# szaguldo-kamaz/FRI-ReinforcementLearning-C

Hardware: AMD Instinct MI355X
Metric: rule-distance evals/sec (rules x envs) (higher is better)
Workload: dtype f64; 1 GPU; cfg4_acrobot_64k_x_8k_per_gpu; nant=5, universe_len=41, rules_per_env=65536, envs_per_gpu=8192, exact_hits=4, dist_backend=none, world_size=1

## Files before the change

### fri-reinforcementlearning-c_amd/__init__.py

```python
import ctypes as C
import os

PKG_DIR = os.path.dirname(os.path.abspath(__file__))
ROOT = os.path.dirname(PKG_DIR)
HIP_LIB_PATH = os.environ.get("FRIRL_HIP_LIB_OVERRIDE") or os.path.join(PKG_DIR, "lib", "libfrirl_hip.so")

NO_HIT = 0xFFFFFFFF
MAX_NANT = 16
MAX_ACTIONS = 32


class FrirlHipError(RuntimeError):
    pass


class Tables(C.Structure):
    _fields_ = [("nant", C.c_int32), ("U", C.c_int32), ("u", C.c_void_p), ("ve", C.c_void_p)]


class RuleBases(C.Structure):
    _fields_ = [("E", C.c_int32), ("maxR", C.c_int32), ("rb", C.c_void_p), ("nrules", C.c_void_p), ("uidx", C.c_void_p)]


MAX_GRID = 64
# ... 29 lines not shown
class ReduceResult(C.Structure):
    _fields_ = [("rules_before", C.c_int32), ("rules_after", C.c_int32), ("rounds", C.c_int32), ("rollouts", C.c_int32),
                ("steps_incremental", C.c_int32), ("reserved", C.c_int32), ("reward", C.c_double)]


class AgentIO(C.Structure):
    _fields_ = [("obs", C.c_void_p), ("q_obs", C.c_void_p), ("reward", C.c_void_p), ("success", C.c_void_p), ("reset", C.c_void_p),
                ("action_out", C.c_void_p), ("action_idx", C.c_void_p)]


class ConvergenceDesc(C.Structure):
    _fields_ = [("prev_nrules", C.c_void_p), ("prev_steps", C.c_void_p), ("prev_reward", C.c_void_p), ("prev_rconc", C.c_void_p),
                ("converged", C.c_void_p), ("episodes", C.c_void_p), ("epended", C.c_void_p)]


_lib = None
_DP = C.POINTER(C.c_double)
LEARN_CHUNK_FN = C.CFUNCTYPE(None, C.c_void_p, C.c_int32, C.c_void_p, C.c_int32)

SIGNATURES = {
    "frirl_hip_version": (C.c_char_p, []),
    "frirl_hip_last_error": (C.c_char_p, []),
    "frirl_hip_device_count": (C.c_int, []),
    "frirl_hip_device_info": (C.c_int, [C.c_int, C.c_char_p, C.c_int, C.POINTER(C.c_int32), C.POINTER(C.c_int64)]),
    "frirl_hip_set_option": (C.c_int, [C.c_char_p, C.c_int]),
    "frirl_hip_get_option": (C.c_int, [C.c_char_p, C.POINTER(C.c_int)]),
    "five_hip_rule_distance_uses_uidx": (C.c_int, [C.c_int32, C.c_int32]),
    "frirl_hip_step_uses_uidx": (C.c_int, [C.c_int32, C.c_int32, C.c_int32, C.c_int32]),
    "five_hip_rule_distance": (C.c_int, [C.POINTER(Tables), C.POINTER(RuleBases), C.c_void_p, C.c_void_p, C.c_void_p, C.c_void_p]),
    "five_hip_rule_distance_packed_words": (C.c_int, [C.c_int32, C.c_int32]),
    "frirl_hip_pack_indices": (C.c_int, [C.POINTER(Tables), C.POINTER(RuleBases), C.c_void_p, C.c_void_p]),
    "five_hip_rule_distance_packed": (C.c_int, [C.POINTER(Tables), C.POINTER(RuleBases), C.c_void_p, C.c_void_p, C.c_void_p, C.c_void_p,
                                                C.c_void_p]),
    "five_hip_sqrt_unscaled_check": (C.c_int, [C.c_void_p, C.c_void_p, C.c_void_p, C.c_int64, C.c_void_p]),
    "five_hip_rule_distance_sq_guard": (C.c_int, [C.POINTER(Tables), C.c_int32, C.c_void_p, C.c_void_p, C.c_void_p]),
    "five_hip_vag_concl": (C.c_int, [C.POINTER(Tables), C.POINTER(RuleBases), C.c_int, C.c_void_p, C.c_void_p, C.c_void_p, C.c_void_p]),
    "five_hip_vag_concl_weight": (C.c_int, [C.POINTER(Tables), C.POINTER(RuleBases), C.c_int, C.c_void_p, C.c_void_p, C.c_void_p, C.c_void_p]),
    "frirl_hip_get_best_action": (C.c_int, [C.POINTER(Tables), C.POINTER(RuleBases), C.c_int, C.c_void_p, C.c_void_p, C.c_int,
                                            C.c_void_p, C.c_void_p, C.c_void_p]),
    "five_hip_vag_concl_shared": (C.c_int, [C.POINTER(Tables), C.POINTER(RuleBases), C.c_int, C.c_int32, C.c_void_p, C.c_void_p, C.c_void_p, C.c_void_p]),
    "frirl_hip_get_best_action_shared": (C.c_int, [C.POINTER(Tables), C.POINTER(RuleBases), C.c_int, C.c_int32, C.c_void_p, C.c_void_p, C.c_int,
                                                   C.c_void_p, C.c_void_p, C.c_void_p]),
    "frirl_hip_rollout_shared": (C.c_int, [C.POINTER(Tables), C.POINTER(RuleBases), C.POINTER(AgentDesc), C.c_int32, C.POINTER(RolloutDesc), C.c_void_p]),
    "frirl_hip_reduce_shared": (C.c_int, [C.POINTER(Tables), C.POINTER(RuleBases), C.POINTER(AgentDesc), C.c_void_p, C.c_int, C.c_double, C.c_int,
                                          C.POINTER(C.c_int32), C.POINTER(ReduceResult), C.c_void_p]),
    "frirl_hip_lanes_preferred": (C.c_int, [C.c_int32, C.c_int32, C.c_int32]),
    "frirl_hip_lanes_workspace_bytes": (C.c_size_t, [C.c_int32, C.c_int32, C.c_int32, C.c_int32]),
    "frirl_hip_episode_run_lanes": (C.c_int, [C.POINTER(Tables), C.POINTER(RuleBases), C.POINTER(AgentDesc), C.POINTER(EnvsDesc), C.c_int32,
                                              C.c_void_p, C.c_size_t, C.c_void_p]),
    "frirl_hip_rollout_resident_rules": (C.c_int, [C.c_int32, C.c_int32, C.c_int32, C.c_int32]),
    "frirl_hip_learn_supported": (C.c_int, [C.c_int32, C.c_int32, C.c_int32, C.c_int32, C.c_int32]),
    "frirl_hip_learn_plan": (C.c_int, [C.c_int32, C.c_int32, C.POINTER(C.c_int32), C.POINTER(C.c_int32)]),
    "frirl_hip_learn_workspace_bytes": (C.c_size_t, [C.c_int32, C.c_int32, C.c_int32, C.c_int32]),
    "frirl_hip_learn_run": (C.c_int, [C.POINTER(Tables), C.POINTER(RuleBases), C.POINTER(AgentDesc), C.POINTER(EnvsDesc), C.POINTER(ConvergenceDesc),
                                      C.c_void_p, C.c_int32, C.c_int32, C.c_int32, C.c_void_p, C.c_void_p, C.c_void_p, C.c_size_t, C.c_void_p]),
    "frirl_hip_learn_train_workspace_bytes": (C.c_size_t, [C.c_int32, C.c_int32, C.c_int32, C.c_int32]),
    "frirl_hip_learn_train": (C.c_int, [C.POINTER(Tables), C.POINTER(RuleBases), C.POINTER(AgentDesc), C.POINTER(EnvsDesc), C.POINTER(ConvergenceDesc),
                                        C.c_int32, C.c_int32, C.c_void_p, C.c_void_p, C.c_void_p, C.c_void_p, C.c_size_t, C.POINTER(C.c_int32),
                                        LEARN_CHUNK_FN, C.c_void_p, C.c_void_p]),
    "five_hip_add_rule": (C.c_int, [C.POINTER(Tables), C.POINTER(RuleBases), C.c_void_p, C.c_void_p, C.c_void_p, C.c_void_p, C.c_void_p,
                                    C.c_void_p]),
    "frirl_hip_update_sarsa": (C.c_int, [C.POINTER(Tables), C.POINTER(RuleBases), C.POINTER(AgentDesc), C.POINTER(EnvsDesc), C.c_void_p,
                                         C.c_void_p, C.c_void_p, C.c_void_p, C.c_void_p]),
    "frirl_hip_env_step": (C.c_int, [C.POINTER(AgentDesc), C.c_int32, C.c_int32, C.c_void_p, C.c_void_p, C.c_void_p, C.c_void_p, C.c_void_p,
                                     C.c_void_p, C.c_void_p]),
    "frirl_hip_episode_begin": (C.c_int, [C.POINTER(Tables), C.POINTER(RuleBases), C.POINTER(AgentDesc), C.POINTER(EnvsDesc), C.c_void_p]),
# ... 89 lines not shown
def _ptr(t):
    return None if t is None else C.c_void_p(t.data_ptr())


def _stream(stream=None):
    import torch
    s = stream if stream is not None else torch.cuda.current_stream()
    return C.c_void_p(s.cuda_stream)


class Problem:

    def __init__(self, u, ve, rb, nrules, uidx=None):
        import torch
        assert u.is_cuda and ve.is_cuda and rb.is_cuda and nrules.is_cuda
        assert u.dtype == torch.float64 and ve.dtype == torch.float64 and rb.dtype == torch.float64 and nrules.dtype == torch.int32
        self.nant, self.U = u.shape
        self.E, cols, self.maxR = rb.shape
        assert cols == self.nant + 1 and ve.shape == u.shape and nrules.shape == (self.E,)
        self.u, self.ve, self.rb, self.nrules = u.contiguous(), ve.contiguous(), rb.contiguous(), nrules.contiguous()
        self.uidx = None
        if uidx is not None:
            assert uidx.is_cuda and uidx.dtype == torch.int16 and uidx.shape == (self.E, self.nant, self.maxR) and self.U <= 32767
            self.uidx = uidx.contiguous()
        self.tables = Tables(self.nant, self.U, self.u.data_ptr(), self.ve.data_ptr())
        self._bases = RuleBases(self.E, self.maxR, self.rb.data_ptr(), self.nrules.data_ptr(),
                                self.uidx.data_ptr() if self.uidx is not None else None)
        self.pidx = None
        self._pidx_key = None
        W = lib().five_hip_rule_distance_packed_words(self.nant, self.U) if self.uidx is not None else 0
        if W > 0:
            self.pidx = torch.empty((self.E, W, self.maxR), dtype=torch.int32, device=self.uidx.device)
            self._pack(None)

    @property
    def bases(self):
        self._pidx_key = None
        return self._bases

    def _pack(self, stream):
        check(lib().frirl_hip_pack_indices(C.byref(self.tables), C.byref(self._bases), _ptr(self.pidx), _stream(stream)),
              "frirl_hip_pack_indices")
        self._pidx_key = (self.uidx.data_ptr(), self.uidx._version)

    def _pidx_current(self, stream):
        if self._pidx_key != (self.uidx.data_ptr(), self.uidx._version):
            self._pack(stream)
        return self.pidx

    def rule_distance(self, x, ruledists=None, hit=None, materialise=True, stream=None):
        import torch
        assert x.is_cuda and x.dtype == torch.float64 and x.shape == (self.E, self.nant) and x.is_contiguous()
        if materialise and ruledists is None:
            ruledists = torch.empty((self.E, self.maxR), dtype=torch.float64, device=x.device)
        if hit is None:
            hit = torch.empty((self.E,), dtype=torch.int32, device=x.device)
        if self.pidx is not None:
            rc = lib().five_hip_rule_distance_packed(C.byref(self.tables), C.byref(self._bases), _ptr(self._pidx_current(stream)), _ptr(x),
                                                     _ptr(ruledists) if materialise else None, _ptr(hit), _stream(stream))
            check(rc, "five_hip_rule_distance_packed")
        else:
            rc = lib().five_hip_rule_distance(C.byref(self.tables), C.byref(self._bases), _ptr(x),
                                              _ptr(ruledists) if materialise else None, _ptr(hit), _stream(stream))
            check(rc, "five_hip_rule_distance")
        return (ruledists if materialise else None), hit

    def vag_concl(self, x, p=0, stream=None):
        import torch
        assert x.is_cuda and x.dtype == torch.float64 and x.shape == (self.E, self.nant) and x.is_contiguous()
        conc = torch.empty((self.E,), dtype=torch.float64, device=x.device)
        hit = torch.empty((self.E,), dtype=torch.int32, device=x.device)
        check(lib().five_hip_vag_concl(C.byref(self.tables), C.byref(self._bases), p, _ptr(x), _ptr(conc), _ptr(hit), _stream(stream)),
              "five_hip_vag_concl")
        return conc, hit

    def vag_concl_weight(self, x, p=0, weights=None, stream=None):
        import torch
        assert x.is_cuda and x.dtype == torch.float64 and x.shape == (self.E, self.nant) and x.is_contiguous()
        if weights is None:
            weights = torch.full((self.E, self.maxR), float("nan"), dtype=torch.float64, device=x.device)
        hit = torch.empty((self.E,), dtype=torch.int32, device=x.device)
        check(lib().five_hip_vag_concl_weight(C.byref(self.tables), C.byref(self._bases), p, _ptr(x), _ptr(weights), _ptr(hit),
                                              _stream(stream)), "five_hip_vag_concl_weight")
        return weights, hit

    def get_best_action(self, states, action_ve, p=0, stream=None):
        import torch
        assert states.is_cuda and states.dtype == torch.float64 and states.shape == (self.E, self.nant - 1) and states.is_contiguous()
        A = action_ve.numel()
        actconc = torch.empty((self.E, A), dtype=torch.float64, device=states.device)
        best = torch.empty((self.E,), dtype=torch.int32, device=states.device)
        check(lib().frirl_hip_get_best_action(C.byref(self.tables), C.byref(self._bases), p, _ptr(states), _ptr(action_ve), A,
                                              _ptr(actconc), _ptr(best), _stream(stream)), "frirl_hip_get_best_action")
# ... 484 lines not shown
```

### fri-reinforcementlearning-c_amd/csrc/device_common.h

```cpp
#pragma once

#include <hip/hip_runtime.h>
#include <stdint.h>

#include "../../include/frirl_hip.h"

#define FRIRL_WAVE 64
#define FRIRL_BLOCK 256
#define FRIRL_WAVES_PER_BLOCK (FRIRL_BLOCK / FRIRL_WAVE)

namespace frirl {

__device__ __forceinline__ unsigned snap_index(const double *__restrict__ uni, int len, double point, double div)
{
    const int low = (int)((point - uni[0]) / div);
    if (low < 0) return 0u;
    if (low >= len) return (unsigned)(len - 1);
    if (low + 1 >= len) return (unsigned)low;
    const double d1 = uni[low] - point;
    const double d2 = uni[low + 1] - point;
    return (fabs(d1) <= fabs(d2)) ? (unsigned)low : (unsigned)(low + 1);
}

__device__ __forceinline__ double universe_div(const double *__restrict__ uni, int U)
// ... 88 lines not shown
    for (int w = 1; w < FRIRL_WAVES_PER_BLOCK; w++) s = s + scratch[w];
    __syncthreads();
    return s;
}

}

namespace frirl_host {
void set_error(const char *fmt, ...);
int check_device();
int check_launch(const char *what);
int check_tables(const frirl_hip_tables *t);
int check_rulebases(const frirl_hip_tables *t, const frirl_hip_rulebases *b);
inline hipStream_t as_stream(void *s) { return reinterpret_cast<hipStream_t>(s); }

struct DeviceGuard {
    int prev = -1;
    DeviceGuard() { if (hipGetDevice(&prev) != hipSuccess) { prev = -1; (void)hipGetLastError(); } }
    ~DeviceGuard() { if (prev >= 0) (void)hipSetDevice(prev); }
    DeviceGuard(const DeviceGuard &) = delete;
    DeviceGuard &operator=(const DeviceGuard &) = delete;
};

struct Options {
    int no_uidx;
    int rd_unroll;
    int rd_chunk;
    int rd_nt;
    int rd_persist;
    int rd_order;
    int rd_packed;
    int rd_sqdiff;
    int rd_qpass;
    int step_wave;
    int step_track;
    int lanes_slices;
    int lanes_wpe;
    int rollout_group;
    int rollout_slices;
    int rollout_resident;
    int rollout_cap;
    int rollout_pair;
    int rollout_wps;
    int learn_slices;
    int learn_alone;
    int learn_persistent;
    int multi_loopback;
    int mirror_sync;
    int no_many;
};
const Options &opts();
}
```

### fri-reinforcementlearning-c_amd/csrc/five_rule_distance.hip

```cpp
#include <stdlib.h>

#include <type_traits>

#include "device_common.h"

namespace frirl {

__device__ __forceinline__ void item_to_env_chunk(unsigned item, int cpe, int E, bool env_fastest, int &e, int &c)
{
    if (env_fastest) { c = (int)(item / (unsigned)E); e = (int)(item - (unsigned)c * (unsigned)E); }
    else { e = (int)(item / (unsigned)cpe); c = (int)(item - (unsigned)e * (unsigned)cpe); }
}

template <int NANT, bool WRITE, int UNROLL, int NT>
__global__ __launch_bounds__(FRIRL_BLOCK) void rule_distance_kernel(
    const double *__restrict__ u, const double *__restrict__ ve, int U, const double *__restrict__ rb,
    const int32_t *__restrict__ nrules, int maxR, const double *__restrict__ x, double *__restrict__ dists,
    uint32_t *__restrict__ hit, int rules_per_block, int cpe, int E, int env_fastest)
{
    int e, c;
    item_to_env_chunk(blockIdx.x, cpe, E, env_fastest != 0, e, c);
    const int R = nrules[e];
    const int r0 = c * rules_per_block;
    if (r0 >= R) return;
// ... 109 lines not shown

    for (int r = r0 + 2 * (int)threadIdx.x; r < r_end; r += STEP * UNROLL) {
        uint32_t w[UNROLL][NANT];
#pragma unroll
        for (int j = 0; j < UNROLL; j++) {
            const int rr = r + j * STEP;
            if (rr < r_end) {
#pragma unroll
                for (int k = 0; k < NANT; k++) w[j][k] = __builtin_nontemporal_load(reinterpret_cast<const uint32_t *>(base + (size_t)k * maxR + rr));
            }
        }
#pragma unroll
        for (int j = 0; j < UNROLL; j++) {
            const int rr = r + j * STEP;
            if (rr < r_end) {
                const double2 d = idx_pair_distance<NANT>(w[j], q, tab_s, U);
                if (WRITE) { __builtin_nontemporal_store(d.x, out + rr); __builtin_nontemporal_store(d.y, out + rr + 1); }
                if (d.y == 0.0 && rr + 1 < R) best = min(best, (unsigned)(rr + 1));
                if (d.x == 0.0) best = min(best, (unsigned)rr);
            }
        }
    }
    best = wave_min_u32(best);
    if ((threadIdx.x & (FRIRL_WAVE - 1)) == 0) red_s[threadIdx.x / FRIRL_WAVE] = best;
    __syncthreads();
    if (threadIdx.x == 0) {
        unsigned m = red_s[0];
        for (int w = 1; w < BLOCK / FRIRL_WAVE; w++) m = red_s[w] < m ? red_s[w] : m;
        if (m != FRIRL_HIP_NO_HIT) atomicMin(&hit[e], m);
    }
}

typedef uint32_t u32x2_t __attribute__((ext_vector_type(2)));

template <int BITS>
__device__ __forceinline__ double pk_table_entry(const double *__restrict__ tab_k, uint32_t w, int sh)
{
    constexpr uint32_t FM = ((1u << BITS) - 1u) << 3;
    const uint32_t off = (sh >= 3 ? (w >> (sh - 3)) : (w << (3 - sh))) & FM;
    return *reinterpret_cast<const double *>(reinterpret_cast<const char *>(tab_k) + off);
}

template <int NANT, int BITS>
__device__ __forceinline__ double2 pk_pair_distance(const u32x2_t (&w)[Packed<BITS>::words(NANT)], const double (&q)[NANT],
                                                    const double *__restrict__ tab_s)
{
    constexpr int FPW = Packed<BITS>::FPW, TS = 1 << BITS;
    double d0 = q[0] - pk_table_entry<BITS>(tab_s, w[0].x, 0), d1 = q[0] - pk_table_entry<BITS>(tab_s, w[0].y, 0);
    double a0 = d0 * d0, a1 = d1 * d1;
#pragma unroll
    for (int k = 1; k < NANT; k++) {
        const int sh = BITS * (k % FPW);
        d0 = q[k] - pk_table_entry<BITS>(tab_s + k * TS, w[k / FPW].x, sh);
        d1 = q[k] - pk_table_entry<BITS>(tab_s + k * TS, w[k / FPW].y, sh);
        const double s0 = d0 * d0, s1 = d1 * d1;
        a0 = a0 + s0;
        a1 = a1 + s1;
    }
    double2 d;
    d.x = __dsqrt_rn(a0);
    d.y = __dsqrt_rn(a1);
    return d;
}

__device__ __forceinline__ double sqrt_unscaled(double x)
{
// ... 11 lines not shown
}

__device__ __forceinline__ bool sq_in_unscaled_range(double s)
{
    return s == 0.0 || (s >= 0x1p-767 && s <= 0x1p1000);
}

template <int NANT, int BITS, bool FAST>
__device__ __forceinline__ void pk_pair_sq(const u32x2_t (&w)[Packed<BITS>::words(NANT)], const double *__restrict__ sq_s, double2 &d,
                                           bool &z0, bool &z1)
{
    constexpr int FPW = Packed<BITS>::FPW, TS = 1 << BITS;
    double a0 = pk_table_entry<BITS>(sq_s, w[0].x, 0), a1 = pk_table_entry<BITS>(sq_s, w[0].y, 0);
#pragma unroll
    for (int k = 1; k < NANT; k++) {
        const int sh = BITS * (k % FPW);
        a0 = a0 + pk_table_entry<BITS>(sq_s + k * TS, w[k / FPW].x, sh);
        a1 = a1 + pk_table_entry<BITS>(sq_s + k * TS, w[k / FPW].y, sh);
    }
    if (FAST) {
        d.x = sqrt_unscaled(a0);
        d.y = sqrt_unscaled(a1);
        z0 = a0 == 0.0;
        z1 = a1 == 0.0;
    } else {
        d.x = __dsqrt_rn(a0);
        d.y = __dsqrt_rn(a1);
        z0 = d.x == 0.0;
        z1 = d.y == 0.0;
    }
}

template <int NANT, int BITS, int BLOCK>
__device__ __forceinline__ bool fill_sq_table(const double *q_s, double *sq_s, const double (&tv)[(NANT * (1 << BITS) + BLOCK - 1) / BLOCK])
{
    constexpr int TS = 1 << BITS, N = NANT * TS;
    bool ok = true;
#pragma unroll
    for (int m = 0; m < (N + BLOCK - 1) / BLOCK; m++) {
        const int i = (int)threadIdx.x + m * BLOCK;
        if (N % BLOCK == 0 || i < N) {
            const double d = q_s[i >> BITS] - tv[m];
            const double s = d * d;
            sq_s[i] = s;
            ok = ok && sq_in_unscaled_range(s);
        }
    }
    return ok;
}

template <int NANT, int BITS, int BLOCK>
__device__ __forceinline__ void load_sq_sources(const double *__restrict__ ve, int U, double (&tv)[(NANT * (1 << BITS) + BLOCK - 1) / BLOCK])
{
    constexpr int TS = 1 << BITS, N = NANT * TS;
#pragma unroll
    for (int m = 0; m < (N + BLOCK - 1) / BLOCK; m++) {
        const int i = (int)threadIdx.x + m * BLOCK;
        const int k = i >> BITS, j = i & (TS - 1);
        tv[m] = (i < N && j < U) ? ve[k * U + j] : 0.0;
    }
}

template <int NANT, bool WRITE, int UNROLL, int BITS, bool SQ>
__global__ __launch_bounds__(FRIRL_BLOCK) void rule_distance_pk_kernel(
    const double *__restrict__ u, const double *__restrict__ ve, int U, const uint32_t *__restrict__ pidx,
    const int32_t *__restrict__ nrules, int maxR, const double *__restrict__ x, const double *__restrict__ qv, double *__restrict__ dists,
    uint32_t *__restrict__ hit, int rules_per_block, int cpe, int E, int env_fastest)
{
    constexpr int W = Packed<BITS>::words(NANT), TS = 1 << BITS;
    __shared__ double tab_s[NANT * TS];
    __shared__ double q_s[NANT];
    __shared__ unsigned red_s[FRIRL_WAVES_PER_BLOCK];
    int e, c;
    item_to_env_chunk(blockIdx.x, cpe, E, env_fastest != 0, e, c);
    const int R = nrules[e];
    const int r0 = c * rules_per_block;
    if (r0 >= R) return;
    int r_end = r0 + rules_per_block;
    if (r_end > R) r_end = R;

    const uint32_t *__restrict__ base = pidx + (size_t)e * W * maxR;
    constexpr int STEP = FRIRL_BLOCK * 2;
    u32x2_t w[UNROLL][W];
    auto load = [&](int r) {
#pragma unroll
        for (int j = 0; j < UNROLL; j++) {
            const int rr = r + j * STEP;
            if (rr < r_end) {
#pragma unroll
                for (int k = 0; k < W; k++) w[j][k] = __builtin_nontemporal_load(reinterpret_cast<const u32x2_t *>(base + (size_t)k * maxR + rr));
            }
        }
    };
    int r = r0 + 2 * (int)threadIdx.x;
    load(r);
    double *__restrict__ out = WRITE ? dists + (size_t)e * maxR : nullptr;
    unsigned best = FRIRL_HIP_NO_HIT;

    if constexpr (SQ) {
        double *sq_s = tab_s;
        double tv[(NANT * TS + FRIRL_BLOCK - 1) / FRIRL_BLOCK];
        load_sq_sources<NANT, BITS, FRIRL_BLOCK>(ve, U, tv);
        if (threadIdx.x < NANT)
            q_s[threadIdx.x] = qv ? qv[(size_t)e * NANT + threadIdx.x] : observe_ve(u, ve, U, threadIdx.x, x[(size_t)e * NANT + threadIdx.x]);
        __syncthreads();
        const bool fast = !__syncthreads_or(!fill_sq_table<NANT, BITS, FRIRL_BLOCK>(q_s, sq_s, tv));
        auto sweep = [&](auto fast_tag) {
            constexpr bool FAST = decltype(fast_tag)::value;
            for (; r < r_end; r += STEP * UNROLL) {
                if (r != r0 + 2 * (int)threadIdx.x) load(r);
#pragma unroll
                for (int j = 0; j < UNROLL; j++) {
                    const int rr = r + j * STEP;
                    if (rr < r_end) {
                        double2 d;
                        bool z0, z1;
                        pk_pair_sq<NANT, BITS, FAST>(w[j], sq_s, d, z0, z1);
                        if (WRITE) { __builtin_nontemporal_store(d.x, out + rr); __builtin_nontemporal_store(d.y, out + rr + 1); }
                        if (z1 && rr + 1 < R) best = min(best, (unsigned)(rr + 1));
                        if (z0) best = min(best, (unsigned)rr);
                    }
                }
            }
        };
        if (fast) sweep(std::true_type{});
        else sweep(std::false_type{});
        best = wave_min_u32(best);
        if ((threadIdx.x & (FRIRL_WAVE - 1)) == 0) red_s[threadIdx.x / FRIRL_WAVE] = best;
        __syncthreads();
        if (threadIdx.x == 0) {
            unsigned m = red_s[0];
            for (int v = 1; v < FRIRL_WAVES_PER_BLOCK; v++) m = red_s[v] < m ? red_s[v] : m;
            if (m != FRIRL_HIP_NO_HIT) atomicMin(&hit[e], m);
        }
        return;
    }

    for (int i = threadIdx.x; i < NANT * TS; i += FRIRL_BLOCK) {
        const int k = i >> BITS, j = i & (TS - 1);
// ... 263 lines not shown
        else VI(UI);
#undef VI
        if (e1 != hipSuccess) { set_error("five_hip_rule_distance: cannot reserve %zu B of LDS: %s", tab_bytes, hipGetErrorString(e1)); return FRIRL_HIP_ELAUNCH; }
        return check_launch("five_hip_rule_distance(uidx)");
    }
    if (!make_grid(b, tn.chunk > 0 ? tn.chunk : (b->maxR <= 16384 + 512 ? 1024 : 2048), g)) { set_error("five_hip_rule_distance: too many work items"); return FRIRL_HIP_EINVAL; }
    if (NANT <= 5 && (tn.unroll || tn.nt >= 0)) {
        const int un = tn.unroll ? tn.unroll : UNROLL;
        const int nt = tn.nt >= 0 ? tn.nt : 1;
#define V(U_, N_) launch_variant<NANT, U_, N_>(t, b, x, ruledists, hit, s, g)
        if (nt == 1) { if (un == 1) V(1, 1); else if (un == 2) V(2, 1); else if (un == 8) V(8, 1); else V(4, 1); }
        else if (nt == 2) { if (un == 1) V(1, 2); else if (un == 2) V(2, 2); else if (un == 8) V(8, 2); else V(4, 2); }
        else if (nt == 3) { if (un == 1) V(1, 3); else if (un == 2) V(2, 3); else if (un == 8) V(8, 3); else V(4, 3); }
        else { if (un == 1) V(1, 0); else if (un == 2) V(2, 0); else if (un == 8) V(8, 0); else V(4, 0); }
#undef V
    } else {
        launch_variant<NANT, UNROLL, 1>(t, b, x, ruledists, hit, s, g);
    }
    return check_launch("five_hip_rule_distance");
}

static constexpr int RD_PK_BITS = 6;

static int packed_words(int nant, int U)
{
    if (nant < 1 || nant > FRIRL_HIP_MAX_NANT || U < 2 || U > (1 << RD_PK_BITS)) return 0;
    if (sizeof(double) * nant * (size_t)U > RD_SMALL_TABLE_BYTES) return 0;
    return Packed<RD_PK_BITS>::words(nant);
}

template <int NANT>
struct RdPkConfig {
    static constexpr int UNROLL = NANT <= 5 ? 8 : 4;
};

template <int NANT, int UN, bool SQ>
static void launch_pk(const frirl_hip_tables *t, const frirl_hip_rulebases *b, const uint32_t *pidx, const double *x, const double *qv,
                      double *ruledists, uint32_t *hit, hipStream_t s, const RdGrid &g)
{
    if (ruledists)
        hipLaunchKernelGGL((rule_distance_pk_kernel<NANT, true, UN, RD_PK_BITS, SQ>), dim3(g.items), dim3(FRIRL_BLOCK), 0, s, t->u, t->ve, t->U, pidx,
                           b->nrules, b->maxR, x, qv, ruledists, hit, g.rules_per_block, g.cpe, b->E, g.env_fastest);
    else
        hipLaunchKernelGGL((rule_distance_pk_kernel<NANT, false, UN, RD_PK_BITS, SQ>), dim3(g.items), dim3(FRIRL_BLOCK), 0, s, t->u, t->ve, t->U, pidx,
                           b->nrules, b->maxR, x, qv, ruledists, hit, g.rules_per_block, g.cpe, b->E, g.env_fastest);
}

template <int NANT, int UN>
static void launch_pk_form(const frirl_hip_tables *t, const frirl_hip_rulebases *b, const uint32_t *pidx, const double *x, const double *qv,
                           double *ruledists, uint32_t *hit, hipStream_t s, const RdGrid &g, bool sq)
{
    if (sq) launch_pk<NANT, UN, true>(t, b, pidx, x, qv, ruledists, hit, s, g);
    else launch_pk<NANT, UN, false>(t, b, pidx, x, nullptr, ruledists, hit, s, g);
}

template <int NANT>
static int launch_packed(const frirl_hip_tables *t, const frirl_hip_rulebases *b, const uint32_t *pidx, const double *x,
                         double *ruledists, uint32_t *hit, hipStream_t s)
{
    using namespace frirl_host;
    constexpr int UP = RdPkConfig<NANT>::UNROLL;
    const RdTune tn = rd_tune();
    const int un = (NANT <= 5 && tn.unroll) ? tn.unroll : UP;
    const bool sq = opts().rd_sqdiff != 0;
    const bool qpass = sq && opts().rd_qpass == 1;
    RdGrid g;
    if (!make_grid(b, tn.chunk > 0 ? tn.chunk : 2 * FRIRL_BLOCK * un, g)) { set_error("five_hip_rule_distance_packed: too many work items"); return FRIRL_HIP_EINVAL; }
    void *scratch = nullptr;
    const double *qv = nullptr;
    if (qpass) {
        const size_t qv_off = 256, bytes = qv_off + sizeof(double) * (size_t)b->E * NANT;
        const hipError_t e1 = hipMallocAsync(&scratch, bytes, s);
        if (e1 != hipSuccess) { (void)hipGetLastError(); set_error("five_hip_rule_distance_packed: hipMallocAsync(%zu B) failed: %s", bytes, hipGetErrorString(e1)); return FRIRL_HIP_ELAUNCH; }
        double *q = reinterpret_cast<double *>(static_cast<char *>(scratch) + qv_off);
        const int nq = b->E * NANT;
        hipLaunchKernelGGL(observe_reset_kernel, dim3((nq + 255) / 256), dim3(256), 0, s, t->u, t->ve, t->U, NANT, b->E, x, q, hit, static_cast<unsigned *>(scratch));
        qv = q;
    } else if (hipMemsetAsync(hit, 0xFF, sizeof(uint32_t) * (size_t)b->E, s) != hipSuccess) {
        return check_launch("five_hip_rule_distance_packed(memset)");
    }
    if constexpr (NANT <= 5) {
        if (un == 4) launch_pk_form<NANT, 4>(t, b, pidx, x, qv, ruledists, hit, s, g, sq);
        else if (un == 2) launch_pk_form<NANT, 2>(t, b, pidx, x, qv, ruledists, hit, s, g, sq);
        else if (un == 1) launch_pk_form<NANT, 1>(t, b, pidx, x, qv, ruledists, hit, s, g, sq);
        else launch_pk_form<NANT, UP>(t, b, pidx, x, qv, ruledists, hit, s, g, sq);
    } else {
        launch_pk_form<NANT, UP>(t, b, pidx, x, qv, ruledists, hit, s, g, sq);
    }
    if (scratch && hipFreeAsync(scratch, s) != hipSuccess) { set_error("five_hip_rule_distance_packed: hipFreeAsync failed"); return FRIRL_HIP_ELAUNCH; }
    return check_launch("five_hip_rule_distance_packed");
}

__global__ void sqrt_unscaled_check_kernel(const double *__restrict__ a, double *__restrict__ fast, double *__restrict__ ref, long n)
{
    const long i = (long)blockIdx.x * blockDim.x + threadIdx.x;
    if (i >= n) return;
    fast[i] = sqrt_unscaled(a[i]);
    ref[i] = __dsqrt_rn(a[i]);
}

template <int NANT>
__global__ __launch_bounds__(FRIRL_BLOCK) void sq_guard_kernel(const double *__restrict__ u, const double *__restrict__ ve, int U,
                                                             const double *__restrict__ x, int32_t *__restrict__ ok)
{
    constexpr int TS = 1 << RD_PK_BITS;
    __shared__ double sq_s[NANT * TS];
    __shared__ double q_s[NANT];
    const int e = blockIdx.x;
    double tv[(NANT * TS + FRIRL_BLOCK - 1) / FRIRL_BLOCK];
    load_sq_sources<NANT, RD_PK_BITS, FRIRL_BLOCK>(ve, U, tv);
    if (threadIdx.x < NANT) q_s[threadIdx.x] = observe_ve(u, ve, U, threadIdx.x, x[(size_t)e * NANT + threadIdx.x]);
    __syncthreads();
    const bool fast = !__syncthreads_or(!fill_sq_table<NANT, RD_PK_BITS, FRIRL_BLOCK>(q_s, sq_s, tv));
    if (threadIdx.x == 0) ok[e] = fast ? 1 : 0;
}

}

extern "C" int five_hip_rule_distance_uses_uidx(int32_t nant, int32_t U)
{
    return nant >= 1 && nant <= FRIRL_HIP_MAX_NANT && U <= 65536 && sizeof(double) * nant * (size_t)U <= 150 * 1024 && !frirl_host::opts().no_uidx;
}

extern "C" int five_hip_rule_distance(const frirl_hip_tables *t, const frirl_hip_rulebases *b, const double *x,
                                      double *ruledists, uint32_t *hit, void *stream)
{
    using namespace frirl_host;
    int rc = check_rulebases(t, b);
    if (rc) return rc;
    if (!x || !hit) { set_error("five_hip_rule_distance: NULL x/hit"); return FRIRL_HIP_EINVAL; }
    if (ruledists && (reinterpret_cast<uintptr_t>(ruledists) & 15)) { set_error("five_hip_rule_distance: ruledists must be 16-byte aligned"); return FRIRL_HIP_EINVAL; }
    if ((rc = check_device())) return rc;
    hipStream_t s = as_stream(stream);

    switch (t->nant) {
#define FRIRL_CASE(N) case N: return frirl::launch_nant<N>(t, b, x, ruledists, hit, s);
        FRIRL_CASE(1) FRIRL_CASE(2) FRIRL_CASE(3) FRIRL_CASE(4) FRIRL_CASE(5) FRIRL_CASE(6) FRIRL_CASE(7) FRIRL_CASE(8)
        FRIRL_CASE(9) FRIRL_CASE(10) FRIRL_CASE(11) FRIRL_CASE(12) FRIRL_CASE(13) FRIRL_CASE(14) FRIRL_CASE(15) FRIRL_CASE(16)
#undef FRIRL_CASE
    }
    set_error("five_hip_rule_distance: unsupported nant=%d", t->nant);
    return FRIRL_HIP_EINVAL;
}

extern "C" int five_hip_rule_distance_packed_words(int32_t nant, int32_t U)
{
// ... 14 lines not shown
    hipLaunchKernelGGL(frirl::pack_indices_kernel<frirl::RD_PK_BITS>, dim3((unsigned)grid), dim3(FRIRL_BLOCK), 0, as_stream(stream), b->uidx, t->nant,
                       b->maxR, total, pidx);
    return check_launch("frirl_hip_pack_indices");
}

extern "C" int five_hip_sqrt_unscaled_check(const double *a, double *fast, double *ref, int64_t n, void *stream)
{
    using namespace frirl_host;
    if (n < 0 || (n && (!a || !fast || !ref))) { set_error("five_hip_sqrt_unscaled_check: bad arguments"); return FRIRL_HIP_EINVAL; }
    int rc = check_device();
    if (rc) return rc;
    if (n) hipLaunchKernelGGL(frirl::sqrt_unscaled_check_kernel, dim3((unsigned)((n + 255) / 256)), dim3(256), 0, as_stream(stream), a, fast, ref, (long)n);
    return check_launch("five_hip_sqrt_unscaled_check");
}

extern "C" int five_hip_rule_distance_sq_guard(const frirl_hip_tables *t, int32_t E, const double *x, int32_t *ok, void *stream)
{
    using namespace frirl_host;
    int rc = check_tables(t);
    if (rc) return rc;
    if (!frirl::packed_words(t->nant, t->U)) { set_error("five_hip_rule_distance_sq_guard: nant=%d U=%d is not served by the packed form", t->nant, t->U); return FRIRL_HIP_EINVAL; }
    if (E < 0 || (E && (!x || !ok))) { set_error("five_hip_rule_distance_sq_guard: bad arguments"); return FRIRL_HIP_EINVAL; }
    if ((rc = check_device())) return rc;
    if (!E) return 0;
    switch (t->nant) {
#define FRIRL_CASE(N) case N: hipLaunchKernelGGL(frirl::sq_guard_kernel<N>, dim3((unsigned)E), dim3(FRIRL_BLOCK), 0, as_stream(stream), t->u, t->ve, t->U, x, ok); break;
        FRIRL_CASE(1) FRIRL_CASE(2) FRIRL_CASE(3) FRIRL_CASE(4) FRIRL_CASE(5) FRIRL_CASE(6) FRIRL_CASE(7) FRIRL_CASE(8)
        FRIRL_CASE(9) FRIRL_CASE(10) FRIRL_CASE(11) FRIRL_CASE(12) FRIRL_CASE(13) FRIRL_CASE(14) FRIRL_CASE(15) FRIRL_CASE(16)
#undef FRIRL_CASE
    }
    return check_launch("five_hip_rule_distance_sq_guard");
}

extern "C" int five_hip_rule_distance_packed(const frirl_hip_tables *t, const frirl_hip_rulebases *b, const uint32_t *pidx, const double *x,
                                             double *ruledists, uint32_t *hit, void *stream)
{
    using namespace frirl_host;
    int rc = check_rulebases(t, b);
    if (rc) return rc;
    const Options &o = opts();
    if (!frirl::packed_words(t->nant, t->U) || !o.rd_packed || o.no_uidx || o.rd_persist == 1)
        return five_hip_rule_distance(t, b, x, ruledists, hit, stream);
    if (!pidx || !x || !hit) { set_error("five_hip_rule_distance_packed: NULL pidx/x/hit"); return FRIRL_HIP_EINVAL; }
    if (reinterpret_cast<uintptr_t>(pidx) & 7) { set_error("five_hip_rule_distance_packed: pidx must be 8-byte aligned"); return FRIRL_HIP_EINVAL; }
    if (ruledists && (reinterpret_cast<uintptr_t>(ruledists) & 15)) { set_error("five_hip_rule_distance_packed: ruledists must be 16-byte aligned"); return FRIRL_HIP_EINVAL; }
    if ((rc = check_device())) return rc;
    hipStream_t s = as_stream(stream);

    switch (t->nant) {
#define FRIRL_CASE(N) case N: return frirl::launch_packed<N>(t, b, pidx, x, ruledists, hit, s);
        FRIRL_CASE(1) FRIRL_CASE(2) FRIRL_CASE(3) FRIRL_CASE(4) FRIRL_CASE(5) FRIRL_CASE(6) FRIRL_CASE(7) FRIRL_CASE(8)
        FRIRL_CASE(9) FRIRL_CASE(10) FRIRL_CASE(11) FRIRL_CASE(12) FRIRL_CASE(13) FRIRL_CASE(14) FRIRL_CASE(15) FRIRL_CASE(16)
#undef FRIRL_CASE
    }
    set_error("five_hip_rule_distance_packed: unsupported nant=%d", t->nant);
    return FRIRL_HIP_EINVAL;
}
```

### fri-reinforcementlearning-c_amd/csrc/runtime.hip

```cpp
#include <stdarg.h>
#include <stdio.h>
#include <stdlib.h>
#include <string.h>

#include <mutex>

#include "device_common.h"

namespace frirl_host {

static thread_local char g_err[512] = "";

void set_error(const char *fmt, ...)
{
    va_list ap;
    va_start(ap, fmt);
    vsnprintf(g_err, sizeof g_err, fmt, ap);
    va_end(ap);
}

static Options g_opts;
static std::once_flag g_opts_once;
struct OptName { const char *name, *env; int Options::*field; int def; };
static const OptName k_opts[] = {
    {"no_uidx", "FRIRL_HIP_NO_UIDX", &Options::no_uidx, 0},
    {"rd_unroll", "FRIRL_HIP_RD_UNROLL", &Options::rd_unroll, 0},
    {"rd_chunk", "FRIRL_HIP_RD_CHUNK", &Options::rd_chunk, 0},
    {"rd_nt", "FRIRL_HIP_RD_NT", &Options::rd_nt, -1},
    {"rd_persist", "FRIRL_HIP_RD_PERSIST", &Options::rd_persist, -1},
    {"rd_order", "FRIRL_HIP_RD_ORDER", &Options::rd_order, 0},
    {"rd_packed", "FRIRL_HIP_RD_PACKED", &Options::rd_packed, 1},
    {"rd_sqdiff", "FRIRL_HIP_RD_SQDIFF", &Options::rd_sqdiff, 1},
    {"rd_qpass", "FRIRL_HIP_RD_QPASS", &Options::rd_qpass, 0},
    {"step_wave", "FRIRL_HIP_STEP_WAVE", &Options::step_wave, -1},
    {"step_track", "FRIRL_HIP_STEP_TRACK", &Options::step_track, -1},
    {"lanes_slices", "FRIRL_HIP_LANES_SLICES", &Options::lanes_slices, 0},
    {"lanes_wpe", "FRIRL_HIP_LANES_WPE", &Options::lanes_wpe, 0},
    {"rollout_group", "FRIRL_HIP_ROLLOUT_GROUP", &Options::rollout_group, 0},
    {"rollout_slices", "FRIRL_HIP_ROLLOUT_SLICES", &Options::rollout_slices, 0},
    {"rollout_resident", "FRIRL_HIP_ROLLOUT_RESIDENT", &Options::rollout_resident, -1},
    {"rollout_cap", "FRIRL_HIP_ROLLOUT_CAP", &Options::rollout_cap, 0},
    {"rollout_pair", "FRIRL_HIP_ROLLOUT_PAIR", &Options::rollout_pair, -1},
    {"rollout_wps", "FRIRL_HIP_ROLLOUT_WPS", &Options::rollout_wps, 0},
    {"learn_slices", "FRIRL_HIP_LEARN_SLICES", &Options::learn_slices, 0},
    {"learn_alone", "FRIRL_HIP_LEARN_ALONE", &Options::learn_alone, 0},
    {"learn_persistent", "FRIRL_HIP_LEARN_PERSISTENT", &Options::learn_persistent, -1},
    {"multi_loopback", "FRIRL_HIP_MULTI_LOOPBACK", &Options::multi_loopback, 0},
    {"no_many", "FRIRL_HIP_NO_MANY", &Options::no_many, 0},
    {"mirror_sync", "FRIRL_HIP_MIRROR_SYNC", &Options::mirror_sync, 0},
};
static void opts_init()
{
    for (const OptName &o : k_opts) {
        const char *e = getenv(o.env);
        g_opts.*(o.field) = e ? atoi(e) : o.def;
    }
}
const Options &opts()
{
    std::call_once(g_opts_once, opts_init);
    return g_opts;
}
static const OptName *find_opt(const char *name)
{
    if (name) for (const OptName &o : k_opts) if (!strcmp(o.name, name)) return &o;
    return nullptr;
// ... 102 lines not shown
```

### include/frirl_hip.h

```cpp
#ifndef FRIRL_HIP_H
#define FRIRL_HIP_H

#include <stdint.h>

#ifdef __cplusplus
extern "C" {
#endif

#define FRIRL_HIP_MAX_NANT     16
#define FRIRL_HIP_MAX_ACTIONS  32
#define FRIRL_HIP_MAX_GRID     64
#define FRIRL_HIP_NO_HIT       0xFFFFFFFFu

#define FRIRL_HIP_ENV_MOUNTAINCAR 0
#define FRIRL_HIP_ENV_CARTPOLE    1
#define FRIRL_HIP_ENV_ACROBOT     2
#define FRIRL_HIP_ENV_EXTERNAL    3

#define FRIRL_HIP_UPD_INACTIVE   0
#define FRIRL_HIP_UPD_EXACT      1
#define FRIRL_HIP_UPD_SPREAD     2
#define FRIRL_HIP_UPD_INSERTED   3
#define FRIRL_HIP_UPD_SKIPPED    4
#define FRIRL_HIP_UPD_FULL       5
// ... 5 lines not shown

typedef struct frirl_hip_tables {
    int32_t nant;
    int32_t U;
    const double *u;
    const double *ve;
} frirl_hip_tables;

typedef struct frirl_hip_rulebases {
    int32_t E;
    int32_t maxR;
    double *rb;
    int32_t *nrules;
    uint16_t *uidx;
} frirl_hip_rulebases;

const char *frirl_hip_version(void);
const char *frirl_hip_last_error(void);
int frirl_hip_device_count(void);
int frirl_hip_device_info(int device, char *name, int name_len, int32_t *cus, int64_t *hbm_bytes);

int frirl_hip_set_option(const char *name, int value);
int frirl_hip_get_option(const char *name, int *value);
int five_hip_rule_distance_uses_uidx(int32_t nant, int32_t U);
int frirl_hip_step_uses_uidx(int32_t nant, int32_t U, int32_t maxR, int32_t E);

int five_hip_rule_distance(const frirl_hip_tables *t, const frirl_hip_rulebases *b, const double *x,
                           double *ruledists, uint32_t *hit, void *stream);

int five_hip_rule_distance_packed_words(int32_t nant, int32_t U);
int frirl_hip_pack_indices(const frirl_hip_tables *t, const frirl_hip_rulebases *b, uint32_t *pidx, void *stream);
int five_hip_rule_distance_packed(const frirl_hip_tables *t, const frirl_hip_rulebases *b, const uint32_t *pidx, const double *x,
                                  double *ruledists, uint32_t *hit, void *stream);
int five_hip_sqrt_unscaled_check(const double *a, double *fast, double *ref, int64_t n, void *stream);
int five_hip_rule_distance_sq_guard(const frirl_hip_tables *t, int32_t E, const double *x, int32_t *ok, void *stream);

int five_hip_vag_concl(const frirl_hip_tables *t, const frirl_hip_rulebases *b, int p, const double *x,
                       double *conc, uint32_t *hit, void *stream);

int five_hip_vag_concl_weight(const frirl_hip_tables *t, const frirl_hip_rulebases *b, int p, const double *x,
                              double *weights, uint32_t *hit, void *stream);

int frirl_hip_get_best_action(const frirl_hip_tables *t, const frirl_hip_rulebases *b, int p, const double *states,
                              const double *action_ve, int A, double *actconc, int32_t *best, void *stream);

typedef struct frirl_hip_agent {
    double alpha, gamma;
    double qdiff_pos_boundary;
    double qdiff_neg_boundary;
    double weight_significant;
    int32_t skip_rules;
    int32_t p;
    int32_t A;
    int32_t env_kind;
    int32_t max_steps;
    int32_t no_random;
    int32_t grid_len[FRIRL_HIP_MAX_NANT];
    double grid_div[FRIRL_HIP_MAX_NANT];
    double values_def[FRIRL_HIP_MAX_NANT];
    const double *grid_values;
    const double *action_ve;
    double epsilon;
    double reward_good_above;
    double qdiff_final_tolerance;
    uint64_t seed;
    int32_t evaluate;
// ... 202 lines not shown
```

Before: 477.4 billion evals/s.

## Precompute per-env squared-difference tables in a pre-pass kernel and reuse across chunks

Adds a separate kernel that builds each environment's squared-difference lookup table and fast-path flag once into a global workspace. The rule-distance kernel then copies that table into LDS with 16-byte loads instead of recomputing it in every block. This removes redundant table construction across the many chunks per env (65536 rules split into chunks). It also adds an XCD-aware block-to-env mapping so chunks of the same env spread across XCDs, and lowers the unroll to 4 for this path. The cost is an extra launch, extra global memory traffic for the workspace, and a cached per-stream workspace allocation on the Python side.

After: 492.4 billion evals/s, median of 6. 3.1% higher.

```diff
diff --git a/fri-reinforcementlearning-c_amd/__init__.py b/fri-reinforcementlearning-c_amd/__init__.py
--- a/fri-reinforcementlearning-c_amd/__init__.py
+++ b/fri-reinforcementlearning-c_amd/__init__.py
@@ -85,6 +85,9 @@
     "frirl_hip_pack_indices": (C.c_int, [C.POINTER(Tables), C.POINTER(RuleBases), C.c_void_p, C.c_void_p]),
     "five_hip_rule_distance_packed": (C.c_int, [C.POINTER(Tables), C.POINTER(RuleBases), C.c_void_p, C.c_void_p, C.c_void_p, C.c_void_p,
                                                 C.c_void_p]),
+    "five_hip_rule_distance_packed_workspace_bytes": (C.c_size_t, [C.c_int32, C.c_int32, C.c_int32]),
+    "five_hip_rule_distance_packed_ws": (C.c_int, [C.POINTER(Tables), C.POINTER(RuleBases), C.c_void_p, C.c_void_p, C.c_void_p, C.c_void_p,
+                                                   C.c_void_p, C.c_size_t, C.c_void_p]),
     "five_hip_sqrt_unscaled_check": (C.c_int, [C.c_void_p, C.c_void_p, C.c_void_p, C.c_int64, C.c_void_p]),
     "five_hip_rule_distance_sq_guard": (C.c_int, [C.POINTER(Tables), C.c_int32, C.c_void_p, C.c_void_p, C.c_void_p]),
     "five_hip_vag_concl": (C.c_int, [C.POINTER(Tables), C.POINTER(RuleBases), C.c_int, C.c_void_p, C.c_void_p, C.c_void_p, C.c_void_p]),
@@ -240,6 +243,7 @@
         if W > 0:
             self.pidx = torch.empty((self.E, W, self.maxR), dtype=torch.int32, device=self.uidx.device)
             self._pack(None)
+        self._rd_ws = {}
 
     @property
     def bases(self):
@@ -255,6 +259,14 @@
         if self._pidx_key != (self.uidx.data_ptr(), self.uidx._version):
             self._pack(stream)
         return self.pidx
+
+    def _rd_workspace(self, stream):
+        import torch
+        key = _stream(stream).value
+        if key not in self._rd_ws:
+            n = lib().five_hip_rule_distance_packed_workspace_bytes(self.nant, self.U, self.E)
+            self._rd_ws[key] = torch.empty((n,), dtype=torch.uint8, device=self.pidx.device) if n else None
+        return self._rd_ws[key]
 
     def rule_distance(self, x, ruledists=None, hit=None, materialise=True, stream=None):
         import torch
@@ -264,9 +276,11 @@
         if hit is None:
             hit = torch.empty((self.E,), dtype=torch.int32, device=x.device)
         if self.pidx is not None:
-            rc = lib().five_hip_rule_distance_packed(C.byref(self.tables), C.byref(self._bases), _ptr(self._pidx_current(stream)), _ptr(x),
-                                                     _ptr(ruledists) if materialise else None, _ptr(hit), _stream(stream))
-            check(rc, "five_hip_rule_distance_packed")
+            ws = self._rd_workspace(stream)
+            rc = lib().five_hip_rule_distance_packed_ws(C.byref(self.tables), C.byref(self._bases), _ptr(self._pidx_current(stream)), _ptr(x),
+                                                        _ptr(ruledists) if materialise else None, _ptr(hit), _ptr(ws),
+                                                        ws.numel() if ws is not None else 0, _stream(stream))
+            check(rc, "five_hip_rule_distance_packed_ws")
         else:
             rc = lib().five_hip_rule_distance(C.byref(self.tables), C.byref(self._bases), _ptr(x),
                                               _ptr(ruledists) if materialise else None, _ptr(hit), _stream(stream))
diff --git a/fri-reinforcementlearning-c_amd/csrc/device_common.h b/fri-reinforcementlearning-c_amd/csrc/device_common.h
--- a/fri-reinforcementlearning-c_amd/csrc/device_common.h
+++ b/fri-reinforcementlearning-c_amd/csrc/device_common.h
@@ -144,6 +144,7 @@
     int rd_packed;
     int rd_sqdiff;
     int rd_qpass;
+    int rd_prepass;
     int step_wave;
     int step_track;
     int lanes_slices;
diff --git a/fri-reinforcementlearning-c_amd/csrc/five_rule_distance.hip b/fri-reinforcementlearning-c_amd/csrc/five_rule_distance.hip
--- a/fri-reinforcementlearning-c_amd/csrc/five_rule_distance.hip
+++ b/fri-reinforcementlearning-c_amd/csrc/five_rule_distance.hip
@@ -165,6 +165,7 @@
 }
 
 typedef uint32_t u32x2_t __attribute__((ext_vector_type(2)));
+static constexpr int RD_XCDS = 8;
 
 template <int BITS>
 __device__ __forceinline__ double pk_table_entry(const double *__restrict__ tab_k, uint32_t w, int sh)
@@ -242,13 +243,13 @@
 }
 
 template <int NANT, int BITS, int BLOCK>
-__device__ __forceinline__ bool fill_sq_table(const double *q_s, double *sq_s, const double (&tv)[(NANT * (1 << BITS) + BLOCK - 1) / BLOCK])
+__device__ __forceinline__ bool fill_sq_table(const double *q_s, double *sq_s, const double (&tv)[(NANT * (1 << BITS) + BLOCK - 1) / BLOCK], int tid)
 {
     constexpr int TS = 1 << BITS, N = NANT * TS;
     bool ok = true;
 #pragma unroll
     for (int m = 0; m < (N + BLOCK - 1) / BLOCK; m++) {
-        const int i = (int)threadIdx.x + m * BLOCK;
+        const int i = tid + m * BLOCK;
         if (N % BLOCK == 0 || i < N) {
             const double d = q_s[i >> BITS] - tv[m];
             const double s = d * d;
@@ -260,29 +261,61 @@
 }
 
 template <int NANT, int BITS, int BLOCK>
-__device__ __forceinline__ void load_sq_sources(const double *__restrict__ ve, int U, double (&tv)[(NANT * (1 << BITS) + BLOCK - 1) / BLOCK])
+__device__ __forceinline__ void load_sq_sources(const double *__restrict__ ve, int U, double (&tv)[(NANT * (1 << BITS) + BLOCK - 1) / BLOCK], int tid)
 {
     constexpr int TS = 1 << BITS, N = NANT * TS;
 #pragma unroll
     for (int m = 0; m < (N + BLOCK - 1) / BLOCK; m++) {
-        const int i = (int)threadIdx.x + m * BLOCK;
+        const int i = tid + m * BLOCK;
         const int k = i >> BITS, j = i & (TS - 1);
         tv[m] = (i < N && j < U) ? ve[k * U + j] : 0.0;
     }
 }
 
-template <int NANT, bool WRITE, int UNROLL, int BITS, bool SQ>
+template <int NANT, int BITS>
+__global__ __launch_bounds__(FRIRL_BLOCK) void sq_tables_kernel(const double *__restrict__ u, const double *__restrict__ ve, int U, int E,
+                                                              const double *__restrict__ x, double *__restrict__ sqtab,
+                                                              uint32_t *__restrict__ fastv, uint32_t *__restrict__ hit)
+{
+    constexpr int TS = 1 << BITS, N = NANT * TS;
+    __shared__ double q_s[FRIRL_WAVES_PER_BLOCK][NANT];
+    const int lane = threadIdx.x & (FRIRL_WAVE - 1), wave = threadIdx.x / FRIRL_WAVE;
+    const int e = blockIdx.x * FRIRL_WAVES_PER_BLOCK + wave;
+    const bool live = e < E;
+    double tv[(N + FRIRL_WAVE - 1) / FRIRL_WAVE];
+    load_sq_sources<NANT, BITS, FRIRL_WAVE>(ve, U, tv, lane);
+    if (live && lane < NANT) q_s[wave][lane] = observe_ve(u, ve, U, lane, x[(size_t)e * NANT + lane]);
+    __syncthreads();
+    if (!live) return;
+    const bool ok = fill_sq_table<NANT, BITS, FRIRL_WAVE>(q_s[wave], sqtab + (size_t)e * N, tv, lane);
+    const bool fast = __all(ok);
+    if (lane == 0) {
+        fastv[e] = fast ? 1u : 0u;
+        hit[e] = FRIRL_HIP_NO_HIT;
+    }
+}
+
+template <int NANT, bool WRITE, int UNROLL, int BITS, bool SQ, bool PRE = false>
 __global__ __launch_bounds__(FRIRL_BLOCK) void rule_distance_pk_kernel(
     const double *__restrict__ u, const double *__restrict__ ve, int U, const uint32_t *__restrict__ pidx,
     const int32_t *__restrict__ nrules, int maxR, const double *__restrict__ x, const double *__restrict__ qv, double *__restrict__ dists,
-    uint32_t *__restrict__ hit, int rules_per_block, int cpe, int E, int env_fastest)
-{
+    uint32_t *__restrict__ hit, int rules_per_block, int cpe, int E, int env_fastest, const double *__restrict__ sqtab = nullptr,
+    const uint32_t *__restrict__ fastv = nullptr)
+{
+    static_assert(SQ || !PRE, "the pre-pass serves the squared-difference form");
     constexpr int W = Packed<BITS>::words(NANT), TS = 1 << BITS;
-    __shared__ double tab_s[NANT * TS];
+    __shared__ __attribute__((aligned(16))) double tab_s[NANT * TS];
     __shared__ double q_s[NANT];
     __shared__ unsigned red_s[FRIRL_WAVES_PER_BLOCK];
     int e, c;
-    item_to_env_chunk(blockIdx.x, cpe, E, env_fastest != 0, e, c);
+    if (PRE && env_fastest == 0) {
+        const unsigned grp = blockIdx.x / (unsigned)(RD_XCDS * cpe), j = blockIdx.x - grp * (unsigned)(RD_XCDS * cpe);
+        e = (int)(grp * RD_XCDS + j % RD_XCDS);
+        c = (int)(j / RD_XCDS);
+        if (e >= E) return;
+    } else {
+        item_to_env_chunk(blockIdx.x, cpe, E, env_fastest == 1, e, c);
+    }
     const int R = nrules[e];
     const int r0 = c * rules_per_block;
     if (r0 >= R) return;
@@ -309,12 +342,21 @@
 
     if constexpr (SQ) {
         double *sq_s = tab_s;
-        double tv[(NANT * TS + FRIRL_BLOCK - 1) / FRIRL_BLOCK];
-        load_sq_sources<NANT, BITS, FRIRL_BLOCK>(ve, U, tv);
-        if (threadIdx.x < NANT)
-            q_s[threadIdx.x] = qv ? qv[(size_t)e * NANT + threadIdx.x] : observe_ve(u, ve, U, threadIdx.x, x[(size_t)e * NANT + threadIdx.x]);
-        __syncthreads();
-        const bool fast = !__syncthreads_or(!fill_sq_table<NANT, BITS, FRIRL_BLOCK>(q_s, sq_s, tv));
+        bool fast;
+        if constexpr (PRE) {
+            constexpr int N2 = NANT * TS / 2;
+            const double2 *__restrict__ src = reinterpret_cast<const double2 *>(sqtab + (size_t)e * (NANT * TS));
+            for (int i = threadIdx.x; i < N2; i += FRIRL_BLOCK) reinterpret_cast<double2 *>(sq_s)[i] = src[i];
+            fast = fastv[e] != 0u;
+            __syncthreads();
+        } else {
+            double tv[(NANT * TS + FRIRL_BLOCK - 1) / FRIRL_BLOCK];
+            load_sq_sources<NANT, BITS, FRIRL_BLOCK>(ve, U, tv, (int)threadIdx.x);
+            if (threadIdx.x < NANT)
+                q_s[threadIdx.x] = qv ? qv[(size_t)e * NANT + threadIdx.x] : observe_ve(u, ve, U, threadIdx.x, x[(size_t)e * NANT + threadIdx.x]);
+            __syncthreads();
+            fast = !__syncthreads_or(!fill_sq_table<NANT, BITS, FRIRL_BLOCK>(q_s, sq_s, tv, (int)threadIdx.x));
+        }
         auto sweep = [&](auto fast_tag) {
             constexpr bool FAST = decltype(fast_tag)::value;
             for (; r < r_end; r += STEP * UNROLL) {
@@ -644,7 +686,14 @@
 template <int NANT>
 struct RdPkConfig {
     static constexpr int UNROLL = NANT <= 5 ? 8 : 4;
+    static constexpr int UNROLL_PRE = 4;
 };
+
+static size_t packed_ws_bytes(int nant, int U, long E)
+{
+    if (!packed_words(nant, U) || E < 1) return 0;
+    return (sizeof(double) * (size_t)nant * (1u << RD_PK_BITS) + sizeof(uint32_t)) * (size_t)E;
+}
 
 template <int NANT, int UN, bool SQ>
 static void launch_pk(const frirl_hip_tables *t, const frirl_hip_rulebases *b, const uint32_t *pidx, const double *x, const double *qv,
@@ -666,18 +715,49 @@
     else launch_pk<NANT, UN, false>(t, b, pidx, x, nullptr, ruledists, hit, s, g);
 }
 
+template <int NANT, int UN>
+static void launch_pk_pre(const frirl_hip_tables *t, const frirl_hip_rulebases *b, const uint32_t *pidx, const double *x, double *ruledists,
+                          uint32_t *hit, void *ws, hipStream_t s, const RdGrid &g)
+{
+    double *sqtab = static_cast<double *>(ws);
+    uint32_t *fastv = reinterpret_cast<uint32_t *>(sqtab + (size_t)b->E * NANT * (1 << RD_PK_BITS));
+    const int order = frirl_host::opts().rd_order;
+    const unsigned items = order == 0 ? (unsigned)g.cpe * (unsigned)((b->E + RD_XCDS - 1) / RD_XCDS * RD_XCDS) : g.items;
+    hipLaunchKernelGGL((sq_tables_kernel<NANT, RD_PK_BITS>), dim3((unsigned)((b->E + FRIRL_WAVES_PER_BLOCK - 1) / FRIRL_WAVES_PER_BLOCK)), dim3(FRIRL_BLOCK),
+                       0, s, t->u, t->ve, t->U, b->E, x, sqtab, fastv, hit);
+    if (ruledists)
+        hipLaunchKernelGGL((rule_distance_pk_kernel<NANT, true, UN, RD_PK_BITS, true, true>), dim3(items), dim3(FRIRL_BLOCK), 0, s, t->u, t->ve, t->U, pidx,
+                           b->nrules, b->maxR, x, nullptr, ruledists, hit, g.rules_per_block, g.cpe, b->E, order, sqtab, fastv);
+    else
+        hipLaunchKernelGGL((rule_distance_pk_kernel<NANT, false, UN, RD_PK_BITS, true, true>), dim3(items), dim3(FRIRL_BLOCK), 0, s, t->u, t->ve, t->U, pidx,
+                           b->nrules, b->maxR, x, nullptr, ruledists, hit, g.rules_per_block, g.cpe, b->E, order, sqtab, fastv);
+}
+
 template <int NANT>
 static int launch_packed(const frirl_hip_tables *t, const frirl_hip_rulebases *b, const uint32_t *pidx, const double *x,
-                         double *ruledists, uint32_t *hit, hipStream_t s)
+                         double *ruledists, uint32_t *hit, void *ws, hipStream_t s)
 {
     using namespace frirl_host;
-    constexpr int UP = RdPkConfig<NANT>::UNROLL;
     const RdTune tn = rd_tune();
+    const bool sq = opts().rd_sqdiff != 0;
+    const bool pre = ws && sq && opts().rd_prepass != 0;
+    const int UP = pre ? RdPkConfig<NANT>::UNROLL_PRE : RdPkConfig<NANT>::UNROLL;
     const int un = (NANT <= 5 && tn.unroll) ? tn.unroll : UP;
-    const bool sq = opts().rd_sqdiff != 0;
-    const bool qpass = sq && opts().rd_qpass == 1;
+    const bool qpass = sq && !pre && opts().rd_qpass == 1;
     RdGrid g;
     if (!make_grid(b, tn.chunk > 0 ? tn.chunk : 2 * FRIRL_BLOCK * un, g)) { set_error("five_hip_rule_distance_packed: too many work items"); return FRIRL_HIP_EINVAL; }
+    if (pre) {
+        if ((long)g.cpe * ((long)b->E + RD_XCDS) > 0x7FFFFFFFL) { set_error("five_hip_rule_distance_packed_ws: too many work items"); return FRIRL_HIP_EINVAL; }
+        if constexpr (NANT <= 5) {
+            if (un == 8) launch_pk_pre<NANT, 8>(t, b, pidx, x, ruledists, hit, ws, s, g);
+            else if (un == 2) launch_pk_pre<NANT, 2>(t, b, pidx, x, ruledists, hit, ws, s, g);
+            else if (un == 1) launch_pk_pre<NANT, 1>(t, b, pidx, x, ruledists, hit, ws, s, g);
+            else launch_pk_pre<NANT, 4>(t, b, pidx, x, ruledists, hit, ws, s, g);
+        } else {
+            launch_pk_pre<NANT, RdPkConfig<NANT>::UNROLL_PRE>(t, b, pidx, x, ruledists, hit, ws, s, g);
+        }
+        return check_launch("five_hip_rule_distance_packed_ws");
+    }
     void *scratch = nullptr;
     const double *qv = nullptr;
     if (qpass) {
@@ -695,9 +775,9 @@
         if (un == 4) launch_pk_form<NANT, 4>(t, b, pidx, x, qv, ruledists, hit, s, g, sq);
         else if (un == 2) launch_pk_form<NANT, 2>(t, b, pidx, x, qv, ruledists, hit, s, g, sq);
         else if (un == 1) launch_pk_form<NANT, 1>(t, b, pidx, x, qv, ruledists, hit, s, g, sq);
-        else launch_pk_form<NANT, UP>(t, b, pidx, x, qv, ruledists, hit, s, g, sq);
+        else launch_pk_form<NANT, RdPkConfig<NANT>::UNROLL>(t, b, pidx, x, qv, ruledists, hit, s, g, sq);
     } else {
-        launch_pk_form<NANT, UP>(t, b, pidx, x, qv, ruledists, hit, s, g, sq);
+        launch_pk_form<NANT, RdPkConfig<NANT>::UNROLL>(t, b, pidx, x, qv, ruledists, hit, s, g, sq);
     }
     if (scratch && hipFreeAsync(scratch, s) != hipSuccess) { set_error("five_hip_rule_distance_packed: hipFreeAsync failed"); return FRIRL_HIP_ELAUNCH; }
     return check_launch("five_hip_rule_distance_packed");
@@ -720,10 +800,10 @@
     __shared__ double q_s[NANT];
     const int e = blockIdx.x;
     double tv[(NANT * TS + FRIRL_BLOCK - 1) / FRIRL_BLOCK];
-    load_sq_sources<NANT, RD_PK_BITS, FRIRL_BLOCK>(ve, U, tv);
+    load_sq_sources<NANT, RD_PK_BITS, FRIRL_BLOCK>(ve, U, tv, (int)threadIdx.x);
     if (threadIdx.x < NANT) q_s[threadIdx.x] = observe_ve(u, ve, U, threadIdx.x, x[(size_t)e * NANT + threadIdx.x]);
     __syncthreads();
-    const bool fast = !__syncthreads_or(!fill_sq_table<NANT, RD_PK_BITS, FRIRL_BLOCK>(q_s, sq_s, tv));
+    const bool fast = !__syncthreads_or(!fill_sq_table<NANT, RD_PK_BITS, FRIRL_BLOCK>(q_s, sq_s, tv, (int)threadIdx.x));
     if (threadIdx.x == 0) ok[e] = fast ? 1 : 0;
 }
 
@@ -804,12 +884,11 @@
     return check_launch("five_hip_rule_distance_sq_guard");
 }
 
-extern "C" int five_hip_rule_distance_packed(const frirl_hip_tables *t, const frirl_hip_rulebases *b, const uint32_t *pidx, const double *x,
-                                             double *ruledists, uint32_t *hit, void *stream)
+static int rule_distance_packed(const frirl_hip_tables *t, const frirl_hip_rulebases *b, const uint32_t *pidx, const double *x,
+                                double *ruledists, uint32_t *hit, void *ws, void *stream)
 {
     using namespace frirl_host;
-    int rc = check_rulebases(t, b);
-    if (rc) return rc;
+    int rc;
     const Options &o = opts();
     if (!frirl::packed_words(t->nant, t->U) || !o.rd_packed || o.no_uidx || o.rd_persist == 1)
         return five_hip_rule_distance(t, b, x, ruledists, hit, stream);
@@ -820,7 +899,7 @@
     hipStream_t s = as_stream(stream);
 
     switch (t->nant) {
-#define FRIRL_CASE(N) case N: return frirl::launch_packed<N>(t, b, pidx, x, ruledists, hit, s);
+#define FRIRL_CASE(N) case N: return frirl::launch_packed<N>(t, b, pidx, x, ruledists, hit, ws, s);
         FRIRL_CASE(1) FRIRL_CASE(2) FRIRL_CASE(3) FRIRL_CASE(4) FRIRL_CASE(5) FRIRL_CASE(6) FRIRL_CASE(7) FRIRL_CASE(8)
         FRIRL_CASE(9) FRIRL_CASE(10) FRIRL_CASE(11) FRIRL_CASE(12) FRIRL_CASE(13) FRIRL_CASE(14) FRIRL_CASE(15) FRIRL_CASE(16)
 #undef FRIRL_CASE
@@ -828,3 +907,33 @@
     set_error("five_hip_rule_distance_packed: unsupported nant=%d", t->nant);
     return FRIRL_HIP_EINVAL;
 }
+
+extern "C" int five_hip_rule_distance_packed(const frirl_hip_tables *t, const frirl_hip_rulebases *b, const uint32_t *pidx, const double *x,
+                                             double *ruledists, uint32_t *hit, void *stream)
+{
+    const int rc = frirl_host::check_rulebases(t, b);
+    return rc ? rc : rule_distance_packed(t, b, pidx, x, ruledists, hit, nullptr, stream);
+}
+
+extern "C" size_t five_hip_rule_distance_packed_workspace_bytes(int32_t nant, int32_t U, int32_t E)
+{
+    return frirl::packed_ws_bytes(nant, U, E);
+}
+
+extern "C" int five_hip_rule_distance_packed_ws(const frirl_hip_tables *t, const frirl_hip_rulebases *b, const uint32_t *pidx, const double *x,
+                                                double *ruledists, uint32_t *hit, void *workspace, size_t workspace_bytes, void *stream)
+{
+    using namespace frirl_host;
+    const int rc = check_rulebases(t, b);
+    if (rc) return rc;
+    const size_t need = frirl::packed_ws_bytes(t->nant, t->U, b->E);
+    if (need) {
+        if (!workspace || workspace_bytes < need) {
+            set_error("five_hip_rule_distance_packed_ws: workspace of %zu B at %p, nant=%d U=%d E=%d needs %zu B "
+                      "(five_hip_rule_distance_packed_workspace_bytes)", workspace_bytes, workspace, t->nant, t->U, b->E, need);
+            return FRIRL_HIP_EINVAL;
+        }
+        if (reinterpret_cast<uintptr_t>(workspace) & 15) { set_error("five_hip_rule_distance_packed_ws: workspace must be 16-byte aligned"); return FRIRL_HIP_EINVAL; }
+    }
+    return rule_distance_packed(t, b, pidx, x, ruledists, hit, need ? workspace : nullptr, stream);
+}
diff --git a/fri-reinforcementlearning-c_amd/csrc/runtime.hip b/fri-reinforcementlearning-c_amd/csrc/runtime.hip
--- a/fri-reinforcementlearning-c_amd/csrc/runtime.hip
+++ b/fri-reinforcementlearning-c_amd/csrc/runtime.hip
@@ -32,6 +32,7 @@
     {"rd_packed", "FRIRL_HIP_RD_PACKED", &Options::rd_packed, 1},
     {"rd_sqdiff", "FRIRL_HIP_RD_SQDIFF", &Options::rd_sqdiff, 1},
     {"rd_qpass", "FRIRL_HIP_RD_QPASS", &Options::rd_qpass, 0},
+    {"rd_prepass", "FRIRL_HIP_RD_PREPASS", &Options::rd_prepass, 1},
     {"step_wave", "FRIRL_HIP_STEP_WAVE", &Options::step_wave, -1},
     {"step_track", "FRIRL_HIP_STEP_TRACK", &Options::step_track, -1},
     {"lanes_slices", "FRIRL_HIP_LANES_SLICES", &Options::lanes_slices, 0},
diff --git a/include/frirl_hip.h b/include/frirl_hip.h
--- a/include/frirl_hip.h
+++ b/include/frirl_hip.h
@@ -61,6 +61,9 @@
 int frirl_hip_pack_indices(const frirl_hip_tables *t, const frirl_hip_rulebases *b, uint32_t *pidx, void *stream);
 int five_hip_rule_distance_packed(const frirl_hip_tables *t, const frirl_hip_rulebases *b, const uint32_t *pidx, const double *x,
                                   double *ruledists, uint32_t *hit, void *stream);
+size_t five_hip_rule_distance_packed_workspace_bytes(int32_t nant, int32_t U, int32_t E);
+int five_hip_rule_distance_packed_ws(const frirl_hip_tables *t, const frirl_hip_rulebases *b, const uint32_t *pidx, const double *x,
+                                     double *ruledists, uint32_t *hit, void *workspace, size_t workspace_bytes, void *stream);
 int five_hip_sqrt_unscaled_check(const double *a, double *fast, double *ref, int64_t n, void *stream);
 int five_hip_rule_distance_sq_guard(const frirl_hip_tables *t, int32_t E, const double *x, int32_t *ok, void *stream);
 
```
